# gorgonia/agogo

Hardware: AMD Instinct MI355X
Metric: mcts_sims_per_sec (higher is better)
Workload: dtype f32 (Winograd F(5x5,3x3): fp32 transforms; transform-domain products as fp16x2 = each fp32 operand scaled by a power of two and split into 2 fp16 pieces (22-23 significand bits, absolute error <= 2^-38 of the tensor range), 3 fp16 MFMAs per product, fp32 accumulate)

## Files before the change

agogo_amd/capi.py:

```python
import ctypes as C
import os

import numpy as np

_HERE = os.path.dirname(os.path.abspath(__file__))
_LIB = None

NONE, BLACK, WHITE = 0, 1, 2
PASS, RESIGN = -1, -2
NO_MOVE = -32768
GAME_MNK, GAME_C4, GAME_KOMI, GAME_WQ = 0, 1, 2, 3
ENC_TWOPLANE, ENC_WQ = 0, 1
INF_NET, INF_DUMMY, INF_SCRIPT, INF_HASH, INF_UNIFORM, INF_CALLBACK = 0, 1, 2, 3, 4, 5
BN_DEGENERATE_EPS, BN_RUNNING, BN_IDENTITY = 0, 1, 2
COMPUTE_F32_MFMA, COMPUTE_BF16X3, COMPUTE_FP16X2, COMPUTE_WINO, COMPUTE_AUTO, COMPUTE_WINO_H2 = 0, 1, 2, 3, 4, 5
COMPUTE_FORCE = 0x100
PROF_CONV, PROF_HEADS, PROF_SELECT, PROF_EXPAND, PROF_MOVE, PROF_CONV_INIT = 0, 1, 2, 3, 4, 5
PROF_WINO_IN, PROF_WINO_GEMM, PROF_WINO_OUT = 6, 7, 8
DONT_PREFER_PASS, PREFER_PASS, DONT_RESIGN = 0, 1, 2
POOL_STRICT, POOL_STOP_SEARCH, POOL_GROW = 0, 1, 2


class AgzError(RuntimeError):
    pass
# ... 171 lines not shown
    sig("agz_arena_drop_labelled_examples", i32, vp)
    sig("agz_arena_examples_dev", i32, vp, pvp, pvp, pvp, pi)
    i64, pi64 = C.c_int64, C.POINTER(C.c_int64)
    sig("agz_train_dev", i32, vp, vp, vp, vp, i32, i32, u64, pf)
    sig("agz_examples_create", i32, vp, i32, i32, i32, i32, pvp)
    sig("agz_examples_destroy", None, vp)
    sig("agz_examples_count", i32, vp, pi64)
    sig("agz_examples_clear", i32, vp)
    sig("agz_examples_append_arena", i32, vp, vp)
    sig("agz_examples_append_dev", i32, vp, vp, vp, vp, i64)
    sig("agz_examples_append_host", i32, vp, pf, pf, pf, i64)
    sig("agz_examples_get", i32, vp, pf, pf, pf, i64, pi64)
    sig("agz_examples_augment_rotate", i32, vp)
    sig("agz_examples_prepare", i32, vp, i32, i32, u64, pi)
    sig("agz_examples_tensors_dev", i32, vp, pvp, pvp, pvp, pi64, pi)
    sig("agz_examples_get_tensors", i32, vp, pf, pf, pf)
    sig("agz_examples_raw_dev", i32, vp, pvp, pvp, pvp)
    sig("agz_rotate_boards", i32, vp, pf, i32, i32, i32, pf)
    sig("agz_ctx_prof_set_stride", i32, vp, i32, i32)
    sig("agz_wino_stages", i32, vp, pf, pf, i32, i32, i32, i32, i32, pf, pf)
    sig("agz_wino_h2_tile", i32, i32, i32)
    sig("agz_net_set_wino_h2_form", i32, vp, i32)
    sig("agz_net_set_wino_h2_gemm", i32, vp, i32)
    sig("agz_net_min_same_batch", i32, vp, i32, i32, C.POINTER(C.c_int))
    sig("agz_arena_set_prep_compact", i32, vp, i32)
    sig("agz_trainer_set_dma_forward", i32, vp, i32)
    sig("agz_arena_last_prep_batch", i32, vp, C.POINTER(C.c_int), C.POINTER(C.c_int))
    sig("agz_arena_debug_counter", i32, vp, i32, C.POINTER(C.c_int64))
    sig("agz_arena_pool_capacity", i32, vp, C.POINTER(C.c_int), C.POINTER(C.c_int))
    sig("agz_wino_h2_chained", i32, i32, i32, i32)
    sig("agz_arena_random_moves", i32, vp, pi, u64)
    sig("agz_arena_set_state", i32, vp, i32, C.POINTER(State))
    sig("agz_arena_examples_labelled_dev", i32, vp, pvp)
    sig("agz_mcts_create", i32, vp, C.POINTER(GameConf), C.POINTER(MctsConf), u64, i32, pvp)
    sig("agz_mcts_destroy", None, vp)
    sig("agz_mcts_set_inferencer", i32, vp, i32, vp)
    sig("agz_mcts_set_inferencer_callback", i32, vp, INFER_FN, vp, i32)
    sig("agz_arena_set_inferencer_callback", i32, vp, i32, INFER_FN, vp, i32)
    sig("agz_arena_set_pool_policy", i32, vp, i32)
    sig("agz_mcts_set_pool_policy", i32, vp, i32)
    sig("agz_mcts_set_parallel", i32, vp, i32)
    sig("agz_mcts_set_game", i32, vp, C.POINTER(State))
    sig("agz_mcts_search", i32, vp, i32, pi)
    sig("agz_mcts_policies", i32, vp, pf, i32)
    sig("agz_mcts_root_children", i32, vp, pi, pu, pf, pf, i32, pi)
    sig("agz_mcts_nodes", i32, vp, pi)
# ... 152 lines not shown
        _check(lib().agz_net_commit(self.h), "agz_net_commit")

    def infer(self, planes):
        c = self.conf
        x = np.ascontiguousarray(planes, dtype=np.float32).reshape(-1, c.Features, c.Height, c.Width)
        B = x.shape[0]
        pol = np.zeros((B, c.ActionSpace), dtype=np.float32)
        val = np.zeros(B, dtype=np.float32)
        _check(lib().agz_net_infer(self.h, _pf(x), B, _pf(pol), _pf(val)), "agz_net_infer")
        return pol, val

    def set_compute_mode(self, mode):
        _check(lib().agz_net_set_compute_mode(self.h, int(mode)), "agz_net_set_compute_mode")

    def set_latency_mode(self, on=True):
        _check(lib().agz_net_set_latency_mode(self.h, int(on)), "agz_net_set_latency_mode")

    def set_tower_queues(self, queues):
        _check(lib().agz_net_set_tower_queues(self.h, int(queues)), "agz_net_set_tower_queues")

    def set_wino_h2_form(self, form):
        _check(lib().agz_net_set_wino_h2_form(self.h, int(form)), "agz_net_set_wino_h2_form")

    def set_wino_h2_gemm(self, variant):
        _check(lib().agz_net_set_wino_h2_gemm(self.h, int(variant)), "agz_net_set_wino_h2_gemm")

    def min_same_batch(self, n, G):
        b = C.c_int(0)
        _check(lib().agz_net_min_same_batch(self.h, int(n), int(G), C.byref(b)), "agz_net_min_same_batch")
        return b.value

    def infer_dev(self, planes_ptr, B, policy_ptr, value_ptr):
        _check(lib().agz_net_infer_dev(self.h, C.c_void_p(planes_ptr), B, C.c_void_p(policy_ptr),
                                       C.c_void_p(value_ptr)), "agz_net_infer_dev")

    def flops_per_eval(self):
        return lib().agz_net_flops_per_eval(self.h)

    def save(self, path):
        _check(lib().agz_net_save(self.h, os.fsencode(path)), "agz_net_save")

    def load(self, path):
        _check(lib().agz_net_load(self.h, os.fsencode(path)), "agz_net_load")


class Trainer:
# ... 609 lines not shown
```

agogo_amd/csrc/conv_wino_h2.hpp:

```cpp
#pragma once

template <int TM> struct WinoT;
template <> struct WinoT<4> {
  static constexpr int AL = 6, VSHIFT = 7;
  static constexpr float BT[6][6] = {{4, 0, -5, 0, 1, 0}, {0, -4, -4, 1, 1, 0}, {0, 4, -4, -1, 1, 0}, {0, -2, -1, 2, 1, 0}, {0, 2, -1, -2, 1, 0}, {0, 4, 0, -5, 0, 1}};
  static constexpr float AT[4][6] = {{1, 1, 1, 1, 1, 0}, {0, 1, -1, 2, -2, 0}, {0, 1, 1, 4, 4, 0}, {0, 1, -1, 8, -8, 1}};
  static constexpr double G[6][3] = {{1.0 / 4, 0, 0}, {-1.0 / 6, -1.0 / 6, -1.0 / 6}, {-1.0 / 6, 1.0 / 6, -1.0 / 6}, {1.0 / 24, 1.0 / 12, 1.0 / 6}, {1.0 / 24, -1.0 / 12, 1.0 / 6}, {0, 0, 1}};
};
template <> struct WinoT<5> {
  static constexpr int AL = 7, VSHIFT = 6;
  static constexpr float BT[7][7] = {{-0.5f, 0.25f, 2.5f, -1.25f, -2, 1, 0}, {0, 0.5f, 0.25f, -2.25f, -1, 1, 0}, {0, -0.5f, 0.75f, 1.75f, -3, 1, 0},
                                     {0, 1, 1.5f, -2, -1.5f, 1, 0},          {0, -1, 2.5f, 0, -2.5f, 1, 0},       {0, 0.25f, 0, -1.25f, 0, 1, 0},
                                     {0, -0.5f, 0.25f, 2.5f, -1.25f, -2, 1}};
  static constexpr float AT[5][7] = {{1, 1, 1, 1, 1, 1, 0}, {0, 1, -1, 0.5f, -0.5f, 2, 0}, {0, 1, 1, 0.25f, 0.25f, 4, 0}, {0, 1, -1, 0.125f, -0.125f, 8, 0},
                                     {0, 1, 1, 0.0625f, 0.0625f, 16, 1}};
  static constexpr double G[7][3] = {{-2, 0, 0}, {-2.0 / 3, -2.0 / 3, -2.0 / 3}, {-2.0 / 9, 2.0 / 9, -2.0 / 9}, {16.0 / 9, 8.0 / 9, 4.0 / 9}, {16.0 / 15, -8.0 / 15, 4.0 / 15},
                                     {2.0 / 45, 4.0 / 45, 8.0 / 45}, {0, 0, 1}};
};
template <int TM> __device__ __forceinline__ void wino_btv(const float* d, float* o);
template <int TM> __device__ __forceinline__ void wino_atv(const float* m, float* o);
template <> __device__ __forceinline__ void wino_btv<4>(const float* d, float* o) { wino_bt6(d, o); }
template <> __device__ __forceinline__ void wino_atv<4>(const float* m, float* o) { wino_at4(m, o); }
template <> __device__ __forceinline__ void wino_btv<5>(const float* d, float* o) {
  o[0] = -0.5f * d[0] + 0.25f * d[1] + 2.5f * d[2] - 1.25f * d[3] - 2.f * d[4] + d[5];
// ... 25 lines not shown
  const float* w_unscale_dev;
  int fuse_prev;
  int wm_per_board;
  unsigned* amax_self;
  int in_swap;
  const _Float16* U2;
  const unsigned* amax_in;
  unsigned* amax_out;
  float* wave_max;
  float w_unscale;
  const float* t_in;
  const float* col_unscale;
  const float* t_next;
  int cform;
  const _Float16* U2c;
  const float* amax_true;
  const float* wm_prev;
  float* wm_out;
  unsigned* amax_next;
  float g1, g0;
  int gemm_variant;
  int temporal_stores;
  int row_pad;
};
__device__ __forceinline__ size_t h2_row(const WinoH2Args& h, int pos, int t) {
  return (size_t)(t >> h.rsh) * h.rA + (size_t)pos * h.rB + (size_t)(t & h.rmask);
}

__device__ __forceinline__ void wino_h2_scales(unsigned amax_bits, int shift, float* s, float* inv) {
  int e = (int)((amax_bits >> 23) & 0xffu);
  if (amax_bits == 0u) { *s = 1.f; *inv = 1.f; return; }
  e = e < 30 ? 30 : (e > 230 ? 230 : e);
  *s = __uint_as_float((unsigned)(268 - shift - e) << 23);
  *inv = __uint_as_float((unsigned)(e - 14 + shift) << 23);
}

__device__ __forceinline__ unsigned wino_h2_pack(float a, float b, unsigned* lo) {
  const _Float16 ha = (_Float16)a, hb = (_Float16)b;
  const _Float16 la = (_Float16)(a - (float)ha), lb = (_Float16)(b - (float)hb);
  *lo = (unsigned)__builtin_bit_cast(unsigned short, la) | ((unsigned)__builtin_bit_cast(unsigned short, lb) << 16);
  return (unsigned)__builtin_bit_cast(unsigned short, ha) | ((unsigned)__builtin_bit_cast(unsigned short, hb) << 16);
}

template <int TM>
__global__ __launch_bounds__(256) void wino_in_h2_kernel(WinoH2Args h) {
  using WT = WinoT<TM>;
// ... 1056 lines not shown
```

agogo_amd/csrc/conv_wino_h2c.hpp:

```cpp
#pragma once

__device__ __forceinline__ unsigned h2c_img(int row, int slot) { return maps::h2c_img(row, slot); }

template <int NK, int PFA>
__global__ __launch_bounds__(256, 2) void wino_gemm_h2c_kernel(WinoH2Args h) {
  const WinoArgs& a = h.w;
  constexpr int SA = 128 * 128, SB = 256 * 128;
  __shared__ __attribute__((aligned(16))) unsigned char lds[SA + SB];

  const int n_nt = a.Ntot >> 8;
  const int per_pos = a.n_mtiles * n_nt;
  const int nblk = h.npos * per_pos;
  const int id = blockIdx.x;
  int q = nblk >> 3, rr = nblk & 7, xcd = id & 7, slot = id >> 3;
  int tile = (xcd < rr ? xcd * (q + 1) : rr * (q + 1) + (xcd - rr) * q) + slot;
  const int pos = tile / per_pos;
  const int rem = tile - pos * per_pos;
  const int m_tile = rem / n_nt, n_tile = rem - m_tile * n_nt;

  const int tid = threadIdx.x, lane = tid & 63, wid = tid >> 6;
  const int wm = wid >> 1, wn = wid & 1;
  const unsigned st_lds = h2c_img(tid >> 3, tid & 7);
  const char* abase = reinterpret_cast<const char*>(a.V) + ((size_t)m_tile * h.npos + pos) * (size_t)NK * SA + (size_t)tid * 16;
  const char* bbase = reinterpret_cast<const char*>(h.U2c) + (((size_t)pos * NK) * n_nt + n_tile) * (size_t)SB + (size_t)tid * 16;
// ... 329 lines not shown
template <int TM> __device__ __forceinline__ void wino_at_acc(int nu, float* Y, float t);
template <> __device__ __forceinline__ void wino_at_acc<5>(int nu, float* Y, float t) {
  switch (nu) {
    case 0: Y[0] += t; break;
    case 1: Y[0] += t; Y[1] += t; Y[2] += t; Y[3] += t; Y[4] += t; break;
    case 2: Y[0] += t; Y[1] -= t; Y[2] += t; Y[3] -= t; Y[4] += t; break;
    case 3: Y[0] += t; Y[1] += 0.5f * t; Y[2] += 0.25f * t; Y[3] += 0.125f * t; Y[4] += 0.0625f * t; break;
    case 4: Y[0] += t; Y[1] -= 0.5f * t; Y[2] += 0.25f * t; Y[3] -= 0.125f * t; Y[4] += 0.0625f * t; break;
    case 5: Y[0] += t; Y[1] += 2.f * t; Y[2] += 4.f * t; Y[3] += 8.f * t; Y[4] += 16.f * t; break;
    default: Y[4] += t; break;
  }
}
template <> __device__ __forceinline__ void wino_at_acc<4>(int nu, float* Y, float t) {
  switch (nu) {
    case 0: Y[0] += t; break;
    case 1: Y[0] += t; Y[1] += t; Y[2] += t; Y[3] += t; break;
    case 2: Y[0] += t; Y[1] -= t; Y[2] += t; Y[3] -= t; break;
    case 3: Y[0] += t; Y[1] += 2.f * t; Y[2] += 4.f * t; Y[3] += 8.f * t; break;
    case 4: Y[0] += t; Y[1] -= 2.f * t; Y[2] += 4.f * t; Y[3] -= 8.f * t; break;
    default: Y[3] += t; break;
  }
}

template <int TM, bool LAST>
__global__ __launch_bounds__(256, 2) void wino_oi_h2c_kernel(WinoH2Args h) {
  using WT = WinoT<TM>;
  constexpr int AL = WT::AL;
  const WinoArgs& a = h.w;
  extern __shared__ __attribute__((aligned(16))) float ys[];
  const int tid = threadIdx.x, tl = tid >> 4, pr = tid & 15, lane = tid & 63;
  const int s = blockIdx.y, NS = a.C >> 5, HW = a.H * a.W;
  const int t0 = blockIdx.x * 16;
  const int t = t0 + tl;
  const bool live = t < a.T;
  const int tc = live ? t : a.T - 1;
  const int b = tc / a.TPB, tt = tc - b * a.TPB;
  const int ty = tt / a.ntx, tx = tt - ty * a.ntx;
  const int bl = tl / a.TPB;
  float s_, un0;
  wino_h2_scales(h.amax_in[b], WT::VSHIFT, &s_, &un0);
  const __amdgpu_buffer_rsrc_t mr = h2_rsrc(a.Mb + ((size_t)(t0 >> 7) * h.npos * NS + s) * 8192);
  const unsigned m_lane = (unsigned)(((tc & 127) * 64 + pr * 4) * 4);
  const unsigned m_pos = (unsigned)NS * 32768u;
  float Y[TM][TM][4];
#pragma unroll
  for (int k = 0; k < TM; k++)
#pragma unroll
    for (int l = 0; l < TM; l++)
// ... 9 lines not shown
      for (int xi = 0; xi < AL; xi++) m[(nu + 1) & 1][xi] = h2_ldf4(mr, m_lane, (unsigned)(xi * AL + nu + 1) * m_pos);
    }
    float mm[4][AL], oo[4][TM];
#pragma unroll
    for (int xi = 0; xi < AL; xi++) { const float4 v = m[nu & 1][xi]; mm[0][xi] = v.x; mm[1][xi] = v.y; mm[2][xi] = v.z; mm[3][xi] = v.w; }
#pragma unroll
    for (int e = 0; e < 4; e++) wino_atv<TM>(mm[e], oo[e]);
#pragma unroll
    for (int k = 0; k < TM; k++)
#pragma unroll
      for (int e = 0; e < 4; e++) {
        float yl[TM];
#pragma unroll
        for (int l = 0; l < TM; l++) yl[l] = Y[k][l][e];
        wino_at_acc<TM>(nu, yl, oo[e][k]);
#pragma unroll
        for (int l = 0; l < TM; l++) Y[k][l][e] = yl[l];
      }
    __builtin_amdgcn_sched_barrier(0);
  }
  const char* ep = reinterpret_cast<const char*>(a.ep);
  const unsigned e_lane = (unsigned)(32 * s + 2 * pr) * 16u, e_pix = (unsigned)a.Cout_p * 16u;
  float mx = 0.f;
  float* yb = LAST ? a.y + (size_t)b * a.Hp * a.Wp * a.Cout_p + 32 * s + 2 * pr : nullptr;
#pragma unroll
  for (int k = 0; k < TM; k++) {
    const int hh = TM * ty + k, hc = hh < a.H ? hh : a.H - 1;
#pragma unroll
    for (int l = 0; l < TM; l++) {
      const int ww = TM * tx + l, wc = ww < a.W ? ww : a.W - 1;
      const char* e = ep + (size_t)(hc * a.W + wc) * e_pix + e_lane;
      const float4 E0 = *reinterpret_cast<const float4*>(e), E1 = *reinterpret_cast<const float4*>(e + 16);
      float va = (Y[k][l][0] * un0) * E0.x + E0.y, vb = (Y[k][l][1] * un0) * E0.z + E0.w;
      float vc = (Y[k][l][2] * un0) * E1.x + E1.y, vd = (Y[k][l][3] * un0) * E1.z + E1.w;
      va = va > 0.f ? va : 0.f; vb = vb > 0.f ? vb : 0.f; vc = vc > 0.f ? vc : 0.f; vd = vd > 0.f ? vd : 0.f;
      const float y0 = va + vb, y1 = vc + vd;
      if (live && hh < a.H && ww < a.W) {
        if (LAST) *reinterpret_cast<float2*>(yb + ((size_t)(hh + 1) * a.Wp + (ww + 1)) * a.Cout_p) = make_float2(y0, y1);
        else *reinterpret_cast<float2*>(&ys[((size_t)bl * HW + hh * a.W + ww) * 32 + 2 * pr]) = make_float2(y0, y1);
        mx = fmaxf(mx, fmaxf(y0, y1));
      }
    }
    __builtin_amdgcn_sched_barrier(0);
  }
  if (LAST) return;
#pragma unroll
  for (int o = 8; o > 0; o >>= 1) mx = fmaxf(mx, __shfl_xor(mx, o, 64));
  if (pr == 0 && live) h.wm_out[(size_t)t * NS + s] = mx;
  float ax;
  if (h.amax_true) ax = __uint_as_float(reinterpret_cast<const unsigned*>(h.amax_true)[b]);
  else {
    const int wmpb = a.TPB * NS;
    const float* wp = h.wm_prev + (size_t)b * wmpb;
    ax = 0.f;
    for (int i = pr; i < wmpb; i += 16) ax = fmaxf(ax, wp[i]);
#pragma unroll
    for (int o = 8; o > 0; o >>= 1) ax = fmaxf(ax, __shfl_xor(ax, o, 64));
  }
  const float bound = h.g1 * ax + h.g0;
  const unsigned bbits = __float_as_uint(bound);
  if (s == 0 && tt == 0 && pr == 0 && live) h.amax_next[b] = bbits;
  float sb, inv_;
  wino_h2_scales(bbits, WT::VSHIFT, &sb, &inv_);
  __syncthreads();
  const float* yl = ys + (size_t)bl * HW * 32 + 2 * pr;
  float tmx[AL][AL], tmy[AL][AL];
// ... 344 lines not shown
      case 1: hipLaunchKernelGGL(wino_gemm_h2p_kernel<1>, gp, dim3(256), 0, st, h); break;
      case 2: hipLaunchKernelGGL(wino_gemm_h2p_kernel<2>, gp, dim3(256), 0, st, h); break;
      case 3: hipLaunchKernelGGL(wino_gemm_h2p_kernel<3>, gp, dim3(256), 0, st, h); break;
      default: hipLaunchKernelGGL(wino_gemm_h2p_kernel<0>, gp, dim3(256), 0, st, h); break;
    }
    return;
  }
  if (dma_ok && h.temporal_stores && (h.w.C >> 5) == 8) { hipLaunchKernelGGL((wino_gemm_h2g_kernel<8, false>), g, dim3(256), 0, st, h); return; }
  if (dma_ok) {
    switch (h.w.C >> 5) {
      case 4: hipLaunchKernelGGL((wino_gemm_h2g_kernel<4>), g, dim3(256), 0, st, h); return;
      case 8: hipLaunchKernelGGL((wino_gemm_h2g_kernel<8>), g, dim3(256), 0, st, h); return;
      case 12: hipLaunchKernelGGL((wino_gemm_h2g_kernel<12>), g, dim3(256), 0, st, h); return;
      default: hipLaunchKernelGGL((wino_gemm_h2g_kernel<16>), g, dim3(256), 0, st, h); return;
    }
  }
  switch (h.w.C >> 5) {
    case 4: hipLaunchKernelGGL((wino_gemm_h2c_kernel<4, 2>), g, dim3(256), 0, st, h); break;
    case 8: hipLaunchKernelGGL((wino_gemm_h2c_kernel<8, 2>), g, dim3(256), 0, st, h); break;
    case 12: hipLaunchKernelGGL((wino_gemm_h2c_kernel<12, 2>), g, dim3(256), 0, st, h); break;
    default: hipLaunchKernelGGL((wino_gemm_h2c_kernel<16, 2>), g, dim3(256), 0, st, h); break;
  }
}
static void wino_h2c_oi(agz_ctx* ctx, WinoH2Args& h, bool last, hipStream_t st, int variant = 4) {
  wino_h2c_geometry(h);
  ProfScopeOn ps(ctx, AGZ_PROF_WINO_OUT, st == ctx->stream);
  const WinoArgs& a = h.w;
  const dim3 g((unsigned)ceil_div(a.T, 16), (unsigned)(a.C >> 5));
  const size_t shm = last ? 0 : (size_t)(16 / a.TPB) * a.H * a.W * 32 * sizeof(float);
  const bool fits31 = wino_h2_rows(h.npos, (size_t)a.T) * a.Ntot * 4 < ((size_t)1 << 31);
  if (variant == 4 && !last && fits31 && !(ctx->func_attr_state & 2u)) {
    const bool ok = hipFuncSetAttribute(reinterpret_cast<const void*>(&wino_oip_h2c_kernel<5>), hipFuncAttributeMaxDynamicSharedMemorySize, 80 * 1024) == hipSuccess &&
                    hipFuncSetAttribute(reinterpret_cast<const void*>(&wino_oip_h2c_kernel<4>), hipFuncAttributeMaxDynamicSharedMemorySize, 80 * 1024) == hipSuccess;
    if (!ok) (void)hipGetLastError();
    ctx->func_attr_state |= 2u | (ok ? 1u : 0u);
  }
  if (variant == 4 && !last && fits31 && (ctx->func_attr_state & 1u)) {
    const size_t shp = (size_t)(16 / a.TPB) * (h.tm * a.nty + 2) * (h.tm * a.ntx + 2) * 32 * sizeof(float);
    const int items = ceil_div(a.T, 16) * (a.C >> 5);
    const dim3 gp((unsigned)std::min(items, 2 * ctx->num_cus));
    if (h.tm == 5 && h.temporal_stores) {
      (void)hipFuncSetAttribute(reinterpret_cast<const void*>(&wino_oip_h2c_kernel<5, false>), hipFuncAttributeMaxDynamicSharedMemorySize, 80 * 1024);
      hipLaunchKernelGGL((wino_oip_h2c_kernel<5, false>), gp, dim3(256), shp, st, h);
      return;
    }
    if (h.tm == 5) hipLaunchKernelGGL((wino_oip_h2c_kernel<5>), gp, dim3(256), shp, st, h);
    else hipLaunchKernelGGL((wino_oip_h2c_kernel<4>), gp, dim3(256), shp, st, h);
    return;
  }
  if (h.tm == 5) {
    if (last) hipLaunchKernelGGL((wino_oi_h2c_kernel<5, true>), g, dim3(256), shm, st, h);
    else hipLaunchKernelGGL((wino_oi_h2c_kernel<5, false>), g, dim3(256), shm, st, h);
  } else {
    if (last) hipLaunchKernelGGL((wino_oi_h2c_kernel<4, true>), g, dim3(256), shm, st, h);
    else hipLaunchKernelGGL((wino_oi_h2c_kernel<4, false>), g, dim3(256), shm, st, h);
  }
}
```

agogo_amd/csrc/net.hip:

```cpp
#include "net.hpp"
#include "gemm_maps.hpp"

#include <cmath>
#include <cstdio>
#include <cstring>
#include <type_traits>

typedef float f32x16 __attribute__((ext_vector_type(16)));
typedef float f32x4 __attribute__((ext_vector_type(4)));

namespace agz {

struct ConvArgs {
  const float* x;
  const float* w;
  const void* ep;
  float* y;
  int M, HW, W, Wp, HpWp;
  int Cin_p, Cout_p, Ntot;
  int n_mtiles, n_ntiles;
  int raw;
  int splits;
  int per;
  float* ws;
// ... 405 lines not shown
  if (p >= a.HW) return;
  int h = p / a.W, w = p - h * a.W;
  const float* xp = a.x + ((size_t)b * a.HpWp + (h + 1) * a.Wp_ + (w + 1)) * a.Kp;
  float s0 = 0.f, s1 = 0.f, s2 = 0.f;
  for (int c = lane * 4; c < a.Kp; c += 256) {
    float4 xv = *reinterpret_cast<const float4*>(xp + c);
    float4 w0 = *reinterpret_cast<const float4*>(a.conv + c);
    float4 w1 = *reinterpret_cast<const float4*>(a.conv + a.Kp + c);
    float4 w2 = *reinterpret_cast<const float4*>(a.conv + 2 * a.Kp + c);
    s0 += xv.x * w0.x + xv.y * w0.y + xv.z * w0.z + xv.w * w0.w;
    s1 += xv.x * w1.x + xv.y * w1.y + xv.z * w1.z + xv.w * w1.w;
    s2 += xv.x * w2.x + xv.y * w2.y + xv.z * w2.z + xv.w * w2.w;
  }
  s0 = wave_sum(s0); s1 = wave_sum(s1); s2 = wave_sum(s2);
  if (lane == 0) {
    float* f = a.feat + (size_t)b * 3 * a.HW;
    float v0 = s0 * a.bn[(0 * a.HW + p) * 2] + a.bn[(0 * a.HW + p) * 2 + 1];
    float v1 = s1 * a.bn[(1 * a.HW + p) * 2] + a.bn[(1 * a.HW + p) * 2 + 1];
    float v2 = s2 * a.bn[(2 * a.HW + p) * 2] + a.bn[(2 * a.HW + p) * 2 + 1];
    f[p] = v0 > 0.f ? v0 : 0.f;
    f[a.HW + p] = v1 > 0.f ? v1 : 0.f;
    f[2 * a.HW + p] = v2 > 0.f ? v2 : 0.f;
  }
}
__global__ __launch_bounds__(1024) void heads_fc_kernel(HeadArgs a) {
  __shared__ float part[16][64];
  const int b = blockIdx.y, lane = threadIdx.x & 63, wv = threadIdx.x >> 6;
  const int col = blockIdx.x * 64 + lane;
  const bool is_pol = col < a.A;
  const int j = is_pol ? col : col - a.A;
  const bool live = col < a.A + a.FC;
  const int rows = is_pol ? 2 * a.HW : a.HW, ld = is_pol ? a.A : a.FC;
  const float* Wm = is_pol ? a.Wp : a.W1;
  const float* f = a.feat + (size_t)b * 3 * a.HW + (is_pol ? 0 : 2 * a.HW);
  const int chunk = (rows + 15) >> 4;
  int i0 = wv * chunk, i1 = i0 + chunk < rows ? i0 + chunk : rows;
  float s = 0.f;
  if (live) {
    int i = i0;
    for (; i + 16 <= i1; i += 16) {
      float fv[16], wv_[16];
#pragma unroll
      for (int u = 0; u < 16; u++) { fv[u] = f[i + u]; wv_[u] = Wm[(size_t)(i + u) * ld + j]; }
#pragma unroll
      for (int u = 0; u < 16; u++) s = fmaf(fv[u], wv_[u], s);
    }
// ... 116 lines not shown
  f(d_w_init); f(d_w_init_t); f(d_ep_init);
  if (d_w3_init) { hipFree(d_w3_init); d_w3_init = nullptr; }
  for (auto& p : d_w_dual) f(p);
  for (auto& p : d_ep_dual) f(p);
  for (auto& p : d_w3_dual) if (p) { hipFree(p); p = nullptr; }
  for (auto& p : d_w2_dual) if (p) { hipFree(p); p = nullptr; }
  if (d_amax) { hipFree(d_amax); d_amax = nullptr; }
  amax_cap = 0;
  for (auto& p : d_u3_dual) if (p) { hipFree(p); p = nullptr; }
  for (auto& p : d_u2_dual) if (p) { hipFree(p); p = nullptr; }
  d_u2_dual.clear();
  for (auto& p : d_u2_tin) if (p) hipFree(p);
  d_u2_tin.clear();
  for (auto& p : d_u2_colun) if (p) hipFree(p);
  d_u2_colun.clear();
  free_u2c();
  for (auto& p : d_ep_h2) if (p) hipFree(p);
  d_ep_h2.clear();
  if (d_ep_init_h2) { hipFree(d_ep_init_h2); d_ep_init_h2 = nullptr; }
  f(d_wV); f(d_wM);
  wino_chunk_cap = 0; wino_v_cap = 0;
  d_w_dual.clear(); d_ep_dual.clear(); d_w3_dual.clear(); d_w2_dual.clear(); d_u3_dual.clear();
  f(d_head_conv); f(d_head_bn); f(d_Wp); f(d_bp); f(d_W1); f(d_b1); f(d_W2); f(d_b2);
  f(d_act_in); f(d_actA); f(d_actB); f(d_planes); f(d_policy); f(d_value); f(d_ws); f(d_hs);
  ws_cap = 0; hs_cap = 0;
  max_batch = 0;
}

int agz_net::ensure_batch(int B) {
  if (B <= max_batch) return AGZ_OK;
  AGZ_REQUIRE((size_t)B * Hp * Wp * (size_t)std::max(Kp, Fp) < ((size_t)1 << 31), AGZ_E_UNSUPPORTED,
              "agz_net: batch %d too large for 32-bit activation offsets (%d x %d board, %d channels)", B, H, W, Kp);
  auto f = [](float*& p) { if (p) { hipFree(p); p = nullptr; } };
  f(d_act_in); f(d_actA); f(d_actB); f(d_planes); f(d_policy); f(d_value);
  size_t px = (size_t)B * Hp * Wp;
  AGZ_HIP_TRY(hipMalloc(&d_act_in, px * Fp * sizeof(float)));
  AGZ_HIP_TRY(hipMalloc(&d_actA, px * Kp * sizeof(float)));
  AGZ_HIP_TRY(hipMalloc(&d_actB, px * Kp * sizeof(float)));
  AGZ_HIP_TRY(hipMalloc(&d_planes, (size_t)B * conf.Features * HW * sizeof(float)));
  AGZ_HIP_TRY(hipMalloc(&d_policy, (size_t)B * conf.ActionSpace * sizeof(float)));
  AGZ_HIP_TRY(hipMalloc(&d_value, (size_t)B * sizeof(float)));
  AGZ_HIP_TRY(hipMemsetAsync(d_act_in, 0, px * Fp * sizeof(float), ctx->stream));
  AGZ_HIP_TRY(hipMemsetAsync(d_actA, 0, px * Kp * sizeof(float), ctx->stream));
  AGZ_HIP_TRY(hipMemsetAsync(d_actB, 0, px * Kp * sizeof(float), ctx->stream));
  max_batch = B;
  return AGZ_OK;
}

// ... 463 lines not shown
    hipLaunchKernelGGL(agz::lat_input_kernel, dim3(Kp / 64, B * in_groups), dim3(256), 0, ctx->stream, li);
    rc = AGZ_OK;
  }
  else if (split_ok && compute_mode != AGZ_COMPUTE_F32_MFMA && d_w3_init && Kp % 128 == 0 &&
      (size_t)B * Hp * Wp * Fp * sizeof(float) < ((size_t)1 << 32)) {
    a.n_ntiles = ceil_div(a.Ntot, 128); a.n_mtiles = ceil_div(a.M, 128);
    a.splits = 1; a.per = 0; a.ws = nullptr; a.raw = 0;
    ProfScope ps(ctx, AGZ_PROF_CONV_INIT);
    if (wino_h2_ok && d_amax && amax_cap >= (size_t)B) {
      AGZ_HIP_TRY(hipMemsetAsync(d_amax, 0, (size_t)B * sizeof(unsigned), ctx->stream));
      a.amax_out = d_amax; amax0_done = true;
    }
    hipLaunchKernelGGL((conv3x3_x3_kernel<false>), dim3(a.n_mtiles * a.n_ntiles), dim3(256), 0, ctx->stream, a, d_w3_init);
    a.amax_out = nullptr;
    rc = AGZ_OK;
  }
  else if (cfg != 0) rc = launch_conv<4, 1, 1, false>(ctx, a, wsp, &ws_cap);
  else if (half_init) rc = launch_conv<2, 2, 1, false>(ctx, a, wsp, &ws_cap);
  else rc = launch_conv<2, 2, 2, false>(ctx, a, wsp, &ws_cap);
  if (rc != AGZ_OK) return rc;
  float* cur = d_actA;
  float* nxt = d_actB;
  bool tower_done = false;
  if (!tower_done && wino_h2_ok) {
    AGZ_REQUIRE((int)d_u2_dual.size() == conf.SharedLayers, AGZ_E_STATE, "agz_net: Winograd fp16x2 weights not built");
    const int npos = (wino_tm + 2) * (wino_tm + 2);
    const int tpb = ceil_div(H, wino_tm) * ceil_div(W, wino_tm);
    const bool wide = plan.wino_wide;
    static const int chunk_env = [] { const char* e = getenv("AGZ_WINO_H2_CHUNK"); return e ? atoi(e) : 0; }();
    static const int queues_env = [] { const char* e = getenv("AGZ_WINO_H2_QUEUES"); return e ? atoi(e) : 0; }();
    const int queues_want = queues_env > 0 ? queues_env : (tower_queues > 0 ? tower_queues : (B >= 256 ? 2 : 1));
    const int chunk_max = (int)std::min<size_t>((size_t)B, ((((size_t)1 << 32) - 1) / ((size_t)npos * Kp * 4) - 127) / tpb);
    int chunk = chunk_env >= 1 ? std::min(chunk_env, chunk_max) : chunk_max;
    const int ns = (queues_want == 2 && B >= 64) ? 2 : 1;
    if (ns == 2 && chunk >= B) chunk = (B + 1) / 2;
    const size_t v_elems = wino_h2_rows(npos, (size_t)chunk * tpb) * Kp, m_elems = 2 * v_elems;
    static const int form_env = [] { const char* e = getenv("AGZ_WINO_H2_FORM"); return e ? atoi(e) : -1; }();
    const int form_want = wino_form >= 0 ? wino_form : form_env;
    const bool chained = form_want != 0 && (int)d_u2c_dual.size() == conf.SharedLayers && agz::wino_h2c_ok(H, W, wino_tm, Kp);
    const int n_scr = chained ? ceil_div(B, chunk) : ns;
    if (v_elems * n_scr > wino_v_cap) {
      AGZ_HIP_TRY(hipStreamSynchronize(ctx->stream));
      if (ctx->stream2) AGZ_HIP_TRY(hipStreamSynchronize(ctx->stream2));
      if (d_wV) hipFree(d_wV);
      if (d_wM) hipFree(d_wM);
      d_wV = d_wM = nullptr; wino_chunk_cap = 0;
      AGZ_HIP_TRY(hipMalloc(&d_wV, v_elems * n_scr * sizeof(float)));
      AGZ_HIP_TRY(hipMalloc(&d_wM, m_elems * n_scr * sizeof(float)));
      wino_v_cap = v_elems * n_scr; wino_chunk_cap = 0;
    }
    const size_t wm_board = chained ? (size_t)tpb * (Kp >> 5) * 2 : (size_t)tpb * (Kp >> 6);
    const size_t need_amax = (size_t)(conf.SharedLayers + 1) * B + wm_board * B;
    if (need_amax > amax_cap) {
      AGZ_HIP_TRY(hipStreamSynchronize(ctx->stream));
      if (ctx->stream2) AGZ_HIP_TRY(hipStreamSynchronize(ctx->stream2));
      if (d_amax) hipFree(d_amax);
      d_amax = nullptr; amax_cap = 0;
      AGZ_HIP_TRY(hipMalloc(&d_amax, need_amax * sizeof(unsigned)));
      amax_cap = need_amax;
      amax0_done = false;
    }
    float* d_wave_max = reinterpret_cast<float*>(d_amax + (size_t)(conf.SharedLayers + 1) * B);
    if (!amax0_done)
// ... 18 lines not shown
        WinoH2Args hh{};
        WinoArgs& wa = hh.w;
        wa.x = cur + (size_t)b0 * Hp * Wp * Kp; wa.y = nxt + (size_t)b0 * Hp * Wp * Kp;
        wa.V = d_wV + (size_t)ci * v_elems; wa.Mb = d_wM + (size_t)ci * m_elems; wa.ep = d_ep_h2[l];
        wa.B = std::min(chunk, B - b0); wa.H = H; wa.W = W; wa.Hp = Hp; wa.Wp = Wp; wa.C = Kp; wa.Cout_p = Kp; wa.Ntot = 2 * Kp;
        hh.U2c = d_u2c_dual[l]; hh.w_unscale = 1.f; hh.tm = wino_tm;
        hh.amax_in = d_amax + (size_t)l * B + b0;
        hh.amax_next = last ? nullptr : d_amax + (size_t)(l + 1) * B + b0;
        hh.amax_true = l == 0 ? reinterpret_cast<const float*>(d_amax + b0) : nullptr;
        hh.wm_prev = d_wave_max + ((size_t)((l + 1) & 1) * B + b0) * wmb;
        hh.wm_out = d_wave_max + ((size_t)(l & 1) * B + b0) * wmb;
        hh.g1 = wino_g1[l]; hh.g0 = wino_g0[l];
        {
          static const int gemm_env = [] {
            const char* e = getenv("AGZ_WINO_H2_GEMM");
            const int v = e ? atoi(e) : 0;
            if (v == 0 || (((v & 63) == 1 || (v & 63) == 2) && (v >> 6) <= 1)) return v;
            fprintf(stderr, "libagz: AGZ_WINO_H2_GEMM=%s ignored (want 1 or 2, optionally + 64)\n", e);
            return 0;
          }();
          const int gv = wino_gemm > 0 ? wino_gemm : gemm_env;
          hh.gemm_variant = gv & 63; hh.temporal_stores = (gv >> 6) & 1;
        }
        if (l == 0) agz::wino_h2c_in(ctx, hh, st);
        agz::wino_h2c_gemm(ctx, hh, st);
        agz::wino_h2c_oi(ctx, hh, last, st, form_want == 1 ? 1 : 4);
      }
      if (last) std::swap(cur, nxt);
    }
    for (int l = 0; !chained && l < conf.SharedLayers; l++) {
      ProfScope ps(ctx, AGZ_PROF_CONV);
      int ci = 0;
      for (int b0 = 0; b0 < B; b0 += chunk, ci++) {
        const int q = ci % ns;
        WinoH2Args hh{};
        WinoArgs& wa = hh.w;
        wa.x = cur + (size_t)b0 * Hp * Wp * Kp; wa.y = nxt + (size_t)b0 * Hp * Wp * Kp;
        wa.V = d_wV + (size_t)q * v_elems; wa.Mb = d_wM + (size_t)q * m_elems; wa.ep = d_ep_h2[l];
        wa.B = std::min(chunk, B - b0); wa.H = H; wa.W = W; wa.Hp = Hp; wa.Wp = Wp; wa.C = Kp; wa.Cout_p = Kp; wa.Ntot = 2 * Kp;
        hh.U2 = d_u2_dual[l]; hh.w_unscale = 1.f; hh.tm = wino_tm;
        hh.t_in = nullptr; hh.col_unscale = nullptr; hh.t_next = nullptr;
        hh.amax_in = d_amax + (size_t)l * B + b0; hh.amax_out = d_amax + (size_t)(l + 1) * B + b0;
        hh.wave_max = d_wave_max + (size_t)b0 * wm_board;
        hh.fuse_prev = l > 0;
        wino_h2_launch(ctx, hh, wide, q ? ctx->stream2 : ctx->stream);
      }
      std::swap(cur, nxt);
    }
    if (ns == 2) {
// ... 73 lines not shown
    else if (cfg != 0) rc = launch_conv<4, 1, 1, true>(ctx, a, wsp, &ws_cap);
    else if (half_dual) rc = launch_conv<2, 2, 1, true>(ctx, a, wsp, &ws_cap);
    else rc = launch_conv<2, 2, 2, true>(ctx, a, wsp, &ws_cap);
    if (rc != AGZ_OK) return rc;
    std::swap(cur, nxt);
  }
  HeadArgs h{};
  h.x = cur; h.conv = d_head_conv; h.bn = d_head_bn; h.Wp = d_Wp; h.bp = d_bp; h.W1 = d_W1; h.b1 = d_b1; h.W2 = d_W2;
  h.b2 = d_b2; h.policy = policy_dev; h.value = value_dev;
  h.H = H; h.W = W; h.HW = HW; h.Wp_ = Wp; h.HpWp = Hp * Wp; h.Kp = Kp; h.A = conf.ActionSpace; h.FC = conf.FC;
  size_t smem = (size_t)(3 * HW + 8 + conf.FC) * sizeof(float);
  {
    ProfScope ps(ctx, AGZ_PROF_HEADS);
    if (heads_spread) {
      size_t need = (size_t)B * (3 * HW + conf.ActionSpace + conf.FC);
      if (need > hs_cap) {
        AGZ_HIP_TRY(hipStreamSynchronize(ctx->stream));
        if (d_hs) hipFree(d_hs);
        d_hs = nullptr; hs_cap = 0;
        AGZ_HIP_TRY(hipMalloc(&d_hs, need * sizeof(float)));
        hs_cap = need;
      }
      h.feat = d_hs; h.cols = d_hs + (size_t)B * 3 * HW;
      hipLaunchKernelGGL(heads_feat_kernel, dim3(ceil_div(HW, 4), B), dim3(256), 0, ctx->stream, h);
      if (plan.heads_nb)
        hipLaunchKernelGGL(heads_fc_nb_kernel<4>, dim3(ceil_div(conf.ActionSpace + conf.FC, 64), ceil_div(B, 4)), dim3(1024), 0, ctx->stream, h, B);
      else
        hipLaunchKernelGGL(heads_fc_kernel, dim3(ceil_div(conf.ActionSpace + conf.FC, 64), B), dim3(1024), 0, ctx->stream, h);
      hipLaunchKernelGGL(heads_out_kernel, dim3(B), dim3(256), 0, ctx->stream, h);
    } else {
      hipLaunchKernelGGL(heads_kernel, dim3(B), dim3(256), smem, ctx->stream, h);
    }
  }
  AGZ_HIP_TRY(hipGetLastError());
  return AGZ_OK;
}

int agz_net::forward_dev(const float* planes_dev, int B, float* policy_dev, float* value_dev) {
  AGZ_REQUIRE(committed, AGZ_E_STATE, "agz_net: infer before agz_net_commit");
  int r = ensure_batch(B);
  if (r != AGZ_OK) return r;
  int total = B * HW * Fp;
  hipLaunchKernelGGL(pack_planes_kernel, dim3(ceil_div(total, 256)), dim3(256), 0, ctx->stream, planes_dev, d_act_in, B,
                     conf.Features, H, W, Fp);
  return forward_packed(B, policy_dev, value_dev);
}

// ... 327 lines not shown
  for (auto& p : n->d_ep_h2) if (p) hipFree(p);
  n->d_ep_h2.clear();
  if (n->d_ep_init_h2) { hipFree(n->d_ep_init_h2); n->d_ep_init_h2 = nullptr; }
  if (n->compute_mode == AGZ_COMPUTE_WINO && n->cfg == 0) return n->build_wino_weights();
  if ((n->compute_mode == AGZ_COMPUTE_WINO_H2 || n->compute_mode == AGZ_COMPUTE_AUTO) && n->cfg == 0) return n->build_wino_h2_weights();
  return AGZ_OK;
}

int agz_wino_h2_tile(int H, int W) { return agz::wino_h2_pick_tm(H, W); }

int agz_wino_h2_chained(int H, int W, int K) {
  static const int form_env = [] { const char* e = getenv("AGZ_WINO_H2_FORM"); return e ? atoi(e) : -1; }();
  const int Kp = agz::round_up(K, 32);
  return form_env != 0 && agz::wino_h2c_ok(H, W, agz::wino_h2_pick_tm(H, W), Kp) ? 1 : 0;
}

int agz_net_set_wino_h2_form(agz_net* n, int form) {
  AGZ_REQUIRE(n, AGZ_E_INVALID, "agz_net_set_wino_h2_form: null net");
  AGZ_REQUIRE(form >= -1 && form <= 2, AGZ_E_INVALID, "agz_net_set_wino_h2_form: form %d (want -1, 0 or 1)", form);
  n->wino_form = form;
  return AGZ_OK;
}

int agz_net_min_same_batch(agz_net* n, int k, int G, int* batch) {
  AGZ_REQUIRE(n && batch && k >= 1 && G >= k, AGZ_E_INVALID, "agz_net_min_same_batch: bad argument");
  AGZ_REQUIRE(n->committed, AGZ_E_STATE, "agz_net_min_same_batch: commit the net first");
  *batch = n->min_same_batch(k, G);
  return AGZ_OK;
}

int agz_net_set_wino_h2_gemm(agz_net* n, int variant) {
  AGZ_REQUIRE(n, AGZ_E_INVALID, "agz_net_set_wino_h2_gemm: null net");
  AGZ_REQUIRE(((variant & 63) <= 2 && (variant >> 6) <= 1) || ((variant & 15) == 2 && (variant >> 4) <= 3), AGZ_E_INVALID, "agz_net_set_wino_h2_gemm: variant %d (want 0, 1, 2, + 64, or 2 + 16 * mode)", variant);
  n->wino_gemm = variant;
  return AGZ_OK;
}

int agz_wino_stages(agz_ctx* ctx, const float* x, const float* w, int B, int H, int W, int C, int N, float* V, float* M) {
  AGZ_REQUIRE(ctx && x && w && V && M, AGZ_E_INVALID, "agz_wino_stages: NULL argument");
  AGZ_REQUIRE(B >= 1 && H >= 1 && W >= 1 && C >= 16 && C % 16 == 0 && N >= 1, AGZ_E_INVALID, "agz_wino_stages: bad shape");
  AGZ_HIP_TRY(hipSetDevice(ctx->device));
  const int Hp = H + 2, Wp = W + 2;
  std::vector<float> xp((size_t)B * Hp * Wp * C, 0.f);
  for (int b = 0; b < B; b++) for (int h = 0; h < H; h++)
    memcpy(&xp[(((size_t)b * Hp + h + 1) * Wp + 1) * C], &x[((size_t)b * H + h) * W * C], (size_t)W * C * sizeof(float));
  std::vector<unsigned short> u3;
// ... 130 lines not shown
```

agogo_amd/csrc/net.hpp:

```cpp
#pragma once
#include <string>
#include <vector>

#include "common.hpp"

namespace agz {
struct Param {
  std::string name;
  std::vector<float> v;
  std::vector<int> ref_shape;
  int kind;
};
struct BNStats { std::vector<float> mean, var; };
int conv3x3_raw(agz_ctx* ctx, const float* x, const float* w, float* y, int B, int H, int W, int Cin_p, int Cout_p);
int conv3x3_raw_x3(agz_ctx* ctx, const float* x, const unsigned short* w3, float* y, int B, int H, int W, int Cin_p, int Cout_p);
int split_w3(agz_ctx* ctx, const float* w, unsigned short* w3, int N, int Cin_p);
inline size_t w3_elems(int N, int Cin_p) { return (size_t)9 * 3 * N * Cin_p; }
struct WinoRawScratch {
  float* V = nullptr; float* M = nullptr; void* U2 = nullptr; unsigned* words = nullptr;
  size_t v_cap = 0, m_cap = 0, u_cap = 0; int b_cap = 0;
  void* w2 = nullptr; unsigned* h2_words = nullptr;
  size_t w2_cap = 0; int h2_b_cap = 0, h2_flip = 0;
};
int conv3x3_raw_h2(agz_ctx* ctx, const float* x, const float* w, float* y, int B, int H, int W, int Cin_p, int Cout_p, WinoRawScratch* sc,
// ... 60 lines not shown
  float* d_b1 = nullptr;
  float* d_W2 = nullptr;
  float* d_b2 = nullptr;

  int max_batch = 0;
  float* d_act_in = nullptr;
  float* d_actA = nullptr;
  float* d_actB = nullptr;
  float* d_planes = nullptr;
  float* d_policy = nullptr;
  float* d_value = nullptr;
  float* d_ws = nullptr;
  std::vector<std::vector<float>> h_ep_dual;
  std::vector<float> h_ep_init;
  std::vector<float*> d_ep_h2;
  float* d_ep_init_h2 = nullptr;
  std::vector<_Float16*> d_lat_w2;
  std::vector<float*> d_lat_tin, d_lat_colun;
  float* d_lat_wmax[2] = {nullptr, nullptr};
  int lat_wmax_cap = 0;
  size_t ws_cap = 0;
  float* d_hs = nullptr;
  size_t hs_cap = 0;
  int tower_queues = 0;
  bool latency_mode = true;

  int ensure_batch(int B);
  void free_device();
  int forward_dev(const float* planes_dev, int B, float* policy_dev, float* value_dev);
  int forward_packed(int B, float* policy_dev, float* value_dev);
  struct FwdPlan { bool half_init, half_dual, small, forced_split, latency, heads_spread, split_ok, heads_nb, wino_wide; };
  FwdPlan fwd_plan(int B) const;
  int min_same_batch(int n, int G) const;
};
```

include/agz_debug.h:

```cpp
#ifndef AGZ_DEBUG_H
#define AGZ_DEBUG_H

#include "agz.h"

#ifdef __cplusplus
extern "C" {
#endif

#define AGZ_PROF_CONV 0
#define AGZ_PROF_HEADS 1
#define AGZ_PROF_SELECT 2
#define AGZ_PROF_EXPAND 3
#define AGZ_PROF_MOVE 4
#define AGZ_PROF_CONV_INIT 5
#define AGZ_PROF_WINO_IN 6
#define AGZ_PROF_WINO_GEMM 7
#define AGZ_PROF_WINO_OUT 8
#define AGZ_PROF_NCLASS 9
int agz_ctx_prof_enable(agz_ctx* ctx, int enable);
int agz_ctx_prof_read(agz_ctx* ctx, int klass, int64_t* launches, double* total_ms);
int agz_ctx_prof_set_stride(agz_ctx* ctx, int klass, int stride);

int agz_wino_stages(agz_ctx* ctx, const float* x, const float* w, int B, int H, int W, int C, int N, float* V, float* M);

int agz_wino_h2_tile(int H, int W);

int agz_wino_h2_chained(int H, int W, int K);

int agz_net_set_wino_h2_form(agz_net* net, int form);

int agz_net_set_wino_h2_gemm(agz_net* net, int variant);

int agz_arena_set_prep_compact(agz_arena* arena, int on);
int agz_arena_last_prep_batch(agz_arena* arena, int* boards, int* roots);

int agz_trainer_set_dma_forward(agz_trainer* t, int on);

int agz_net_min_same_batch(agz_net* net, int n, int G, int* batch);

#define AGZ_CNT_PATHMAX 15
int agz_arena_debug_counter(agz_arena* arena, int which, int64_t* value);

int agz_arena_pool_capacity(agz_arena* arena, int* nodes_per_pool, int* grows);

int agz_comm_debug_fail_slice(agz_comm* comm, int k);

int agz_comm_debug_fail_layer(agz_comm* comm, int layer);

#ifdef __cplusplus
}
#endif
#endif
```

Measured before the change: 43350.

## Fuse head 1x1 conv partial sums into last Winograd output kernel

```diff
diff --git a/agogo_amd/capi.py b/agogo_amd/capi.py
--- a/agogo_amd/capi.py
+++ b/agogo_amd/capi.py
@@ -217,6 +217,7 @@
     sig("agz_wino_h2_tile", i32, i32, i32)
     sig("agz_net_set_wino_h2_form", i32, vp, i32)
     sig("agz_net_set_wino_h2_gemm", i32, vp, i32)
+    sig("agz_net_set_wino_h2_ends", i32, vp, i32)
     sig("agz_net_min_same_batch", i32, vp, i32, i32, C.POINTER(C.c_int))
     sig("agz_arena_set_prep_compact", i32, vp, i32)
     sig("agz_trainer_set_dma_forward", i32, vp, i32)
@@ -415,6 +416,9 @@
     def set_wino_h2_form(self, form):
         _check(lib().agz_net_set_wino_h2_form(self.h, int(form)), "agz_net_set_wino_h2_form")
 
+    def set_wino_h2_ends(self, mask):
+        _check(lib().agz_net_set_wino_h2_ends(self.h, int(mask)), "agz_net_set_wino_h2_ends")
+
     def set_wino_h2_gemm(self, variant):
         _check(lib().agz_net_set_wino_h2_gemm(self.h, int(variant)), "agz_net_set_wino_h2_gemm")
 
diff --git a/agogo_amd/csrc/conv_wino_h2.hpp b/agogo_amd/csrc/conv_wino_h2.hpp
--- a/agogo_amd/csrc/conv_wino_h2.hpp
+++ b/agogo_amd/csrc/conv_wino_h2.hpp
@@ -71,6 +71,8 @@
   int gemm_variant;
   int temporal_stores;
   int row_pad;
+  const float* head_conv;
+  float* head_part;
 };
 __device__ __forceinline__ size_t h2_row(const WinoH2Args& h, int pos, int t) {
   return (size_t)(t >> h.rsh) * h.rA + (size_t)pos * h.rB + (size_t)(t & h.rmask);
diff --git a/agogo_amd/csrc/conv_wino_h2c.hpp b/agogo_amd/csrc/conv_wino_h2c.hpp
--- a/agogo_amd/csrc/conv_wino_h2c.hpp
+++ b/agogo_amd/csrc/conv_wino_h2c.hpp
@@ -375,8 +375,10 @@
   }
 }
 
-template <int TM, bool LAST>
+constexpr int HEADF_LD = 36;
+template <int TM, bool LAST, bool HEADF = false>
 __global__ __launch_bounds__(256, 2) void wino_oi_h2c_kernel(WinoH2Args h) {
+  static_assert(LAST || !HEADF, "the head features replace the last block's y");
   using WT = WinoT<TM>;
   constexpr int AL = WT::AL;
   const WinoArgs& a = h.w;
@@ -432,7 +434,7 @@
   const char* ep = reinterpret_cast<const char*>(a.ep);
   const unsigned e_lane = (unsigned)(32 * s + 2 * pr) * 16u, e_pix = (unsigned)a.Cout_p * 16u;
   float mx = 0.f;
-  float* yb = LAST ? a.y + (size_t)b * a.Hp * a.Wp * a.Cout_p + 32 * s + 2 * pr : nullptr;
+  float* yb = LAST && !HEADF ? a.y + (size_t)b * a.Hp * a.Wp * a.Cout_p + 32 * s + 2 * pr : nullptr;
 #pragma unroll
   for (int k = 0; k < TM; k++) {
     const int hh = TM * ty + k, hc = hh < a.H ? hh : a.H - 1;
@@ -446,12 +448,38 @@
       va = va > 0.f ? va : 0.f; vb = vb > 0.f ? vb : 0.f; vc = vc > 0.f ? vc : 0.f; vd = vd > 0.f ? vd : 0.f;
       const float y0 = va + vb, y1 = vc + vd;
       if (live && hh < a.H && ww < a.W) {
-        if (LAST) *reinterpret_cast<float2*>(yb + ((size_t)(hh + 1) * a.Wp + (ww + 1)) * a.Cout_p) = make_float2(y0, y1);
+        if (HEADF) *reinterpret_cast<float2*>(&ys[((size_t)bl * HW + hh * a.W + ww) * HEADF_LD + 2 * pr]) = make_float2(y0, y1);
+        else if (LAST) *reinterpret_cast<float2*>(yb + ((size_t)(hh + 1) * a.Wp + (ww + 1)) * a.Cout_p) = make_float2(y0, y1);
         else *reinterpret_cast<float2*>(&ys[((size_t)bl * HW + hh * a.W + ww) * 32 + 2 * pr]) = make_float2(y0, y1);
         mx = fmaxf(mx, fmaxf(y0, y1));
       }
     }
     __builtin_amdgcn_sched_barrier(0);
+  }
+  if (HEADF) {
+    __syncthreads();
+    const int b_first = t0 / a.TPB, n_pix = (16 / a.TPB) * HW;
+    const float* hw = h.head_conv + 32 * s;
+    for (int idx = tid; idx < n_pix; idx += 256) {
+      const int b2 = idx / HW, p = idx - b2 * HW;
+      if (b_first + b2 >= a.B) break;
+      const float4* yp = reinterpret_cast<const float4*>(ys + (size_t)idx * HEADF_LD);
+      float s0 = 0.f, s1 = 0.f, s2 = 0.f;
+#pragma unroll
+      for (int q = 0; q < 8; q++) {
+        const float4 v = yp[q];
+        const float e[4] = {v.x, v.y, v.z, v.w};
+#pragma unroll
+        for (int c = 0; c < 4; c++) {
+          s0 = fmaf(e[c], hw[4 * q + c], s0);
+          s1 = fmaf(e[c], hw[a.C + 4 * q + c], s1);
+          s2 = fmaf(e[c], hw[2 * a.C + 4 * q + c], s2);
+        }
+      }
+      float* d = h.head_part + ((size_t)(b_first + b2) * NS + s) * 3 * HW + p;
+      d[0] = s0; d[HW] = s1; d[2 * HW] = s2;
+    }
+    return;
   }
   if (LAST) return;
 #pragma unroll
@@ -842,7 +870,11 @@
     default: hipLaunchKernelGGL((wino_gemm_h2c_kernel<16, 2>), g, dim3(256), 0, st, h); break;
   }
 }
-static void wino_h2c_oi(agz_ctx* ctx, WinoH2Args& h, bool last, hipStream_t st, int variant = 4) {
+static inline size_t wino_h2c_headf_lds(int H, int W, int tm) {
+  return (size_t)(16 / (ceil_div(H, tm) * ceil_div(W, tm))) * H * W * HEADF_LD * sizeof(float);
+}
+static inline bool wino_h2c_headf_ok(int H, int W, int tm) { return wino_h2c_headf_lds(H, W, tm) <= 64 * 1024; }
+static void wino_h2c_oi(agz_ctx* ctx, WinoH2Args& h, bool last, hipStream_t st, int variant = 4, bool headf = false) {
   wino_h2c_geometry(h);
   ProfScopeOn ps(ctx, AGZ_PROF_WINO_OUT, st == ctx->stream);
   const WinoArgs& a = h.w;
@@ -868,6 +900,12 @@
     else hipLaunchKernelGGL((wino_oip_h2c_kernel<4>), gp, dim3(256), shp, st, h);
     return;
   }
+  if (last && headf) {
+    const size_t shh = wino_h2c_headf_lds(a.H, a.W, h.tm);
+    if (h.tm == 5) hipLaunchKernelGGL((wino_oi_h2c_kernel<5, true, true>), g, dim3(256), shh, st, h);
+    else hipLaunchKernelGGL((wino_oi_h2c_kernel<4, true, true>), g, dim3(256), shh, st, h);
+    return;
+  }
   if (h.tm == 5) {
     if (last) hipLaunchKernelGGL((wino_oi_h2c_kernel<5, true>), g, dim3(256), shm, st, h);
     else hipLaunchKernelGGL((wino_oi_h2c_kernel<5, false>), g, dim3(256), shm, st, h);
diff --git a/agogo_amd/csrc/net.hip b/agogo_amd/csrc/net.hip
--- a/agogo_amd/csrc/net.hip
+++ b/agogo_amd/csrc/net.hip
@@ -451,6 +451,16 @@
     f[a.HW + p] = v1 > 0.f ? v1 : 0.f;
     f[2 * a.HW + p] = v2 > 0.f ? v2 : 0.f;
   }
+}
+__global__ __launch_bounds__(256) void heads_feat_part_kernel(HeadArgs a, const float* part, int NS, int n) {
+  const int idx = blockIdx.x * 256 + threadIdx.x;
+  if (idx >= n) return;
+  const int per = 3 * a.HW, b = idx / per, r = idx - b * per;
+  const float* p = part + (size_t)b * NS * per + r;
+  float s = p[0];
+  for (int q = 1; q < NS; q++) s += p[(size_t)q * per];
+  const float v = s * a.bn[r * 2] + a.bn[r * 2 + 1];
+  a.feat[(size_t)b * per + r] = v > 0.f ? v : 0.f;
 }
 __global__ __launch_bounds__(1024) void heads_fc_kernel(HeadArgs a) {
   __shared__ float part[16][64];
@@ -613,8 +623,8 @@
   wino_chunk_cap = 0; wino_v_cap = 0;
   d_w_dual.clear(); d_ep_dual.clear(); d_w3_dual.clear(); d_w2_dual.clear(); d_u3_dual.clear();
   f(d_head_conv); f(d_head_bn); f(d_Wp); f(d_bp); f(d_W1); f(d_b1); f(d_W2); f(d_b2);
-  f(d_act_in); f(d_actA); f(d_actB); f(d_planes); f(d_policy); f(d_value); f(d_ws); f(d_hs);
-  ws_cap = 0; hs_cap = 0;
+  f(d_act_in); f(d_actA); f(d_actB); f(d_planes); f(d_policy); f(d_value); f(d_ws); f(d_hs); f(d_hpart);
+  ws_cap = 0; hs_cap = 0; hpart_cap = 0;
   max_batch = 0;
 }
 
@@ -1124,6 +1134,7 @@
   float* cur = d_actA;
   float* nxt = d_actB;
   bool tower_done = false;
+  bool heads_from_part = false;
   if (!tower_done && wino_h2_ok) {
     AGZ_REQUIRE((int)d_u2_dual.size() == conf.SharedLayers, AGZ_E_STATE, "agz_net: Winograd fp16x2 weights not built");
     const int npos = (wino_tm + 2) * (wino_tm + 2);
@@ -1141,6 +1152,19 @@
     const int form_want = wino_form >= 0 ? wino_form : form_env;
     const bool chained = form_want != 0 && (int)d_u2c_dual.size() == conf.SharedLayers && agz::wino_h2c_ok(H, W, wino_tm, Kp);
     const int n_scr = chained ? ceil_div(B, chunk) : ns;
+    const int ends = wino_ends >= 0 ? wino_ends : 3;
+    heads_from_part = chained && (ends & 2) && heads_spread && conf.SharedLayers > 0 && agz::wino_h2c_headf_ok(H, W, wino_tm);
+    if (heads_from_part) {
+      const size_t need = (size_t)B * (Kp >> 5) * 3 * HW;
+      if (need > hpart_cap) {
+        AGZ_HIP_TRY(hipStreamSynchronize(ctx->stream));
+        if (ctx->stream2) AGZ_HIP_TRY(hipStreamSynchronize(ctx->stream2));
+        if (d_hpart) hipFree(d_hpart);
+        d_hpart = nullptr; hpart_cap = 0;
+        AGZ_HIP_TRY(hipMalloc(&d_hpart, need * sizeof(float)));
+        hpart_cap = need;
+      }
+    }
     if (v_elems * n_scr > wino_v_cap) {
       AGZ_HIP_TRY(hipStreamSynchronize(ctx->stream));
       if (ctx->stream2) AGZ_HIP_TRY(hipStreamSynchronize(ctx->stream2));
@@ -1205,9 +1229,10 @@
           const int gv = wino_gemm > 0 ? wino_gemm : gemm_env;
           hh.gemm_variant = gv & 63; hh.temporal_stores = (gv >> 6) & 1;
         }
+        if (last && heads_from_part) { hh.head_conv = d_head_conv; hh.head_part = d_hpart + (size_t)b0 * (Kp >> 5) * 3 * HW; }
         if (l == 0) agz::wino_h2c_in(ctx, hh, st);
         agz::wino_h2c_gemm(ctx, hh, st);
-        agz::wino_h2c_oi(ctx, hh, last, st, form_want == 1 ? 1 : 4);
+        agz::wino_h2c_oi(ctx, hh, last, st, form_want == 1 ? 1 : 4, last && heads_from_part);
       }
       if (last) std::swap(cur, nxt);
     }
@@ -1327,7 +1352,12 @@
         hs_cap = need;
       }
       h.feat = d_hs; h.cols = d_hs + (size_t)B * 3 * HW;
-      hipLaunchKernelGGL(heads_feat_kernel, dim3(ceil_div(HW, 4), B), dim3(256), 0, ctx->stream, h);
+      if (heads_from_part) {
+        const int n = B * 3 * HW;
+        hipLaunchKernelGGL(heads_feat_part_kernel, dim3(ceil_div(n, 256)), dim3(256), 0, ctx->stream, h, (const float*)d_hpart, Kp >> 5, n);
+      } else {
+        hipLaunchKernelGGL(heads_feat_kernel, dim3(ceil_div(HW, 4), B), dim3(256), 0, ctx->stream, h);
+      }
       if (plan.heads_nb)
         hipLaunchKernelGGL(heads_fc_nb_kernel<4>, dim3(ceil_div(conf.ActionSpace + conf.FC, 64), ceil_div(B, 4)), dim3(1024), 0, ctx->stream, h, B);
       else
@@ -1701,6 +1731,12 @@
   return AGZ_OK;
 }
 
+int agz_net_set_wino_h2_ends(agz_net* n, int mask) {
+  AGZ_REQUIRE(n, AGZ_E_INVALID, "agz_net_set_wino_h2_ends: null net");
+  AGZ_REQUIRE(mask >= -1 && mask <= 3, AGZ_E_INVALID, "agz_net_set_wino_h2_ends: mask %d (want -1 or 0 .. 3)", mask);
+  n->wino_ends = mask;
+  return AGZ_OK;
+}
 int agz_net_min_same_batch(agz_net* n, int k, int G, int* batch) {
   AGZ_REQUIRE(n && batch && k >= 1 && G >= k, AGZ_E_INVALID, "agz_net_min_same_batch: bad argument");
   AGZ_REQUIRE(n->committed, AGZ_E_STATE, "agz_net_min_same_batch: commit the net first");
diff --git a/agogo_amd/csrc/net.hpp b/agogo_amd/csrc/net.hpp
--- a/agogo_amd/csrc/net.hpp
+++ b/agogo_amd/csrc/net.hpp
@@ -106,6 +106,9 @@
   size_t ws_cap = 0;
   float* d_hs = nullptr;
   size_t hs_cap = 0;
+  float* d_hpart = nullptr;
+  size_t hpart_cap = 0;
+  int wino_ends = -1;
   int tower_queues = 0;
   bool latency_mode = true;
 
diff --git a/include/agz_debug.h b/include/agz_debug.h
--- a/include/agz_debug.h
+++ b/include/agz_debug.h
@@ -31,6 +31,8 @@
 
 int agz_net_set_wino_h2_gemm(agz_net* net, int variant);
 
+int agz_net_set_wino_h2_ends(agz_net* net, int mask);
+
 int agz_arena_set_prep_compact(agz_arena* arena, int on);
 int agz_arena_last_prep_batch(agz_arena* arena, int* boards, int* roots);
 
```

Result: no change. 43820, median of 6 (+1.1%).
